# turtle-robotics/sea-current

Measured on AMD Instinct MI355X. Metric: plans/sec (batched start-goal, 1024^2 grid), higher is better.
Workload: dtype int32; 1 GPU; 1024x1024 random-obstacle grids (salt20, one grid and one query block per step), EDT + A*, 1024 batched queries per GPU and step, 10 steps = 10240 queries per library call; queries_per_launch=10240, map=salt20, queries_per_gpu=1024, queries_total=1024, lmax=4096, parallelism=query-sharded x1, contexts_in_flight=2, steps_per_call=10, hw_queues=4

## Files before the change

### sea-current_amd/csrc/astar.hip

```cpp
#include "sc_internal.h"
#include <stdlib.h>

#define NBUCKET 32
#define ASTAR_CQ_THROUGHPUT 1024
#define ASTAR_RU_THROUGHPUT 4
#define ASTAR_CQ_LATENCY 2048
#define ASTAR_RU_LATENCY 8
#define E_RUN (1u << 18)
#define E_START (4u << 13 | 3u << 16)
#define RUNK 8

struct astar_args {
    const uint8_t* moves;
    const int32_t* d2;
    int W, H;
    int32_t rmin;
    const int32_t* start;
    const int32_t* goal;
    const int32_t* qgrid;
    const int32_t* order;
    const int32_t* nq_dev;
    int nq;
    int Lmax;
    int32_t* path;
// ... 11 lines not shown
    int32_t* ovf_sticky;
    int nstat;
    int lazy;
    int tw, bw;
    size_t gcells, bwords;
};

__device__ __forceinline__ int octile(int x, int y, int gx, int gy) {
    int dx = abs(x - gx), dy = abs(y - gy);
    return 10 * max(dx, dy) + 4 * min(dx, dy);
}

__device__ __forceinline__ uint32_t gix(int x, int y, int tw) {
    return ((((uint32_t)(y >> 2) * (uint32_t)tw + (uint32_t)(x >> 2)) << 4) | ((uint32_t)(y & 3) << 2)) | (uint32_t)(x & 3);
}
__device__ __forceinline__ uint32_t gix8(int x, int y, int tw8) {
    return ((((uint32_t)(y >> 3) * (uint32_t)tw8 + (uint32_t)(x >> 3)) << 6) | ((uint32_t)(y & 7) << 3)) | (uint32_t)(x & 7);
}
template <typename GT> __device__ __forceinline__ uint32_t gidx(int x, int y, int tw);
template <> __device__ __forceinline__ uint32_t gidx<uint32_t>(int x, int y, int tw) { return gix(x, y, tw); }
template <> __device__ __forceinline__ uint32_t gidx<uint8_t>(int x, int y, int tw) { return gix8(x, y, tw); }
__device__ __forceinline__ uint32_t cix(int x, int y, int bw) {
    return (((uint32_t)(y >> 4) * (uint32_t)bw + (uint32_t)(x >> 5)) << 4) | (uint32_t)(y & 15);
}

template <typename T>
__device__ __forceinline__ T g_load(const T* p) {
    return __hip_atomic_load(p, __ATOMIC_RELAXED, __HIP_MEMORY_SCOPE_AGENT);
}

__device__ __forceinline__ uint32_t prune_always(int d) {
    const unsigned long long T = 0x75B6D9EA34C851A2ull;
    return (uint32_t)(T >> (8 * d)) & 0xFFu;
}

__device__ __forceinline__ uint32_t entry_pack(int x, int y, int d, uint32_t pmv) {
    const int e0 = (int)((0x6476u >> (4 * (d & 3))) & 7u), e1 = (int)((0x7554u >> (4 * (d & 3))) & 7u);
    const uint32_t side = d < 4 ? (((pmv >> e0) & 1u) | (((pmv >> e1) & 1u) << 1)) : 0u;
// ... 24 lines not shown
                 : "vcc", "scc", "memory");
}
__device__ __forceinline__ void atomic_wait(uint32_t& old) { asm volatile("s_waitcnt vmcnt(0)" : "+v"(old) : : "memory"); }
__device__ __forceinline__ void pop_pair_issue(const uint8_t* mv_addr, uint32_t* bit_addr, uint32_t bits, uint32_t& pmv, uint32_t& old) {
    unsigned long long sv;
    asm volatile("global_load_ubyte %[m], %[ma], off\n\t"
                 "s_mov_b64 %[sv], exec\n\t"
                 "v_cmp_ne_u32_e32 vcc, 0, %[b]\n\t"
                 "s_and_b64 exec, %[sv], vcc\n\t"
                 "global_atomic_or %[o], %[a], %[b], off sc0\n\t"
                 "s_mov_b64 exec, %[sv]"
                 : [sv] "=&s"(sv), [o] "+v"(old), [m] "=&v"(pmv)
                 : [a] "v"(bit_addr), [b] "v"(bits), [ma] "v"(mv_addr)
                 : "vcc", "scc", "memory");
}
__device__ __forceinline__ void pop_run_issue(const uint8_t* const (&ra)[RUNK - 1], const uint8_t* mv_addr, uint32_t* bit_addr, uint32_t bits,
                                              uint32_t (&rm)[RUNK - 1], uint32_t& pmv, uint32_t& old) {
    static_assert(RUNK == 8, "seven run loads are spelled out");
    unsigned long long sv;
    asm volatile("global_load_ubyte %[r0], %[p0], off\n\t"
                 "global_load_ubyte %[r1], %[p1], off\n\t"
                 "global_load_ubyte %[r2], %[p2], off\n\t"
                 "global_load_ubyte %[r3], %[p3], off\n\t"
                 "global_load_ubyte %[r4], %[p4], off\n\t"
                 "global_load_ubyte %[r5], %[p5], off\n\t"
                 "global_load_ubyte %[r6], %[p6], off\n\t"
                 "global_load_ubyte %[m], %[ma], off\n\t"
                 "s_mov_b64 %[sv], exec\n\t"
                 "v_cmp_ne_u32_e32 vcc, 0, %[b]\n\t"
                 "s_and_b64 exec, %[sv], vcc\n\t"
                 "global_atomic_or %[o], %[a], %[b], off sc0\n\t"
                 "s_mov_b64 exec, %[sv]"
                 : [sv] "=&s"(sv), [o] "+v"(old), [m] "=&v"(pmv), [r0] "=&v"(rm[0]), [r1] "=&v"(rm[1]), [r2] "=&v"(rm[2]), [r3] "=&v"(rm[3]),
                   [r4] "=&v"(rm[4]), [r5] "=&v"(rm[5]), [r6] "=&v"(rm[6])
                 : [a] "v"(bit_addr), [b] "v"(bits), [ma] "v"(mv_addr), [p0] "v"(ra[0]), [p1] "v"(ra[1]), [p2] "v"(ra[2]), [p3] "v"(ra[3]),
                   [p4] "v"(ra[4]), [p5] "v"(ra[5]), [p6] "v"(ra[6])
                 : "vcc", "scc", "memory");
}
__device__ __forceinline__ void pop_run_wait_loads(uint32_t (&rm)[RUNK - 1], uint32_t& pmv, uint32_t& old) {
    asm volatile("s_waitcnt vmcnt(1)" : "+v"(pmv), "+v"(old), "+v"(rm[0]), "+v"(rm[1]), "+v"(rm[2]), "+v"(rm[3]), "+v"(rm[4]), "+v"(rm[5]), "+v"(rm[6]) : : "memory");
}
__device__ __forceinline__ void pop_pair_wait_load(uint32_t& pmv, uint32_t& old) { asm volatile("s_waitcnt vmcnt(1)" : "+v"(pmv), "+v"(old) : : "memory"); }

__device__ __forceinline__ void pop_loads_issue(const uint8_t* mv_addr, const uint32_t* w_addr, uint32_t& byte, uint32_t& word) {
    asm volatile("global_load_ubyte %0, %2, off\n\t"
                 "global_load_dword %1, %3, off sc1"
                 : "=&v"(byte), "=&v"(word) : "v"(mv_addr), "v"(w_addr) : "memory");
}
__device__ __forceinline__ void pop_loads_wait(uint32_t& byte, uint32_t& word) { asm volatile("s_waitcnt vmcnt(0)" : "+v"(byte), "+v"(word) : : "memory"); }
__device__ __forceinline__ void masked_or_noret(uint32_t* addr, uint32_t bits) {
// ... 25 lines not shown
    __shared__ uint16_t succ[512];
    __shared__ uint8_t prune_tbl[64];
    __shared__ uint32_t dup_tbl[DUAL ? 1024 + 64 : 1];
    __shared__ uint2 hq_rec[DUAL ? HQ + 64 : 1];
    __shared__ int hq_tail, hq_head, hq_clean, hq_stop, hq_ovf, hq_fcur, hq_found, hq_flush;
    constexpr int SCOPE = DUAL ? __HIP_MEMORY_SCOPE_WORKGROUP : __HIP_MEMORY_SCOPE_WAVEFRONT;
    const int lane = threadIdx.x & 63;
    const int wv = DUAL ? __builtin_amdgcn_readfirstlane((int)(threadIdx.x >> 6)) : 0;
    const int W = a.W, H = a.H;
    const size_t cells = (size_t)W * H;
    const int s = a.start[q], t = a.goal[q];
    int32_t* path = a.path + (size_t)q * a.Lmax;

    int out_st = SC_Q_OK, out_len = 0, out_cost = -1, nexp = 0, npop = 0, kcyc = 0, nstep = 0;
    const size_t grid_off = a.qgrid ? (size_t)a.qgrid[q] * cells : 0;
    const uint8_t* const mvs = a.moves + grid_off;
    const bool bad = s < 0 || t < 0 || (size_t)s >= cells || (size_t)t >= cells || a.d2[grid_off + s] < a.rmin || a.d2[grid_off + t] < a.rmin;
    if (bad) out_st = SC_Q_BAD_ENDPOINT;
    else if (s == t) {
        if (lane == 0 && wv == 0) path[0] = s;
        out_len = 1; out_cost = 0; nexp = 1;
    } else {
    const int tw = a.tw, bw = a.bw;
    GT* g = static_cast<GT*>(a.g) + (size_t)slot * a.gcells;
    uint32_t* cl = a.closed + (size_t)slot * a.bwords;
    uint32_t* bk = a.buckets + (size_t)slot * NBUCKET * a.cap;
    const int cap = a.cap, capm = a.cap - 1;
    const int sx = s % W, sy = s / W, gx = t % W, gy = t / W;
    const int ddx[8] = {1, -1, 0, 0, 1, -1, 1, -1};
    const int ddy[8] = {0, 0, 1, -1, 1, 1, -1, -1};

    {
        uint4* p = reinterpret_cast<uint4*>(cl);
        const size_t n4 = a.bwords >> 2;
        for (size_t i = DUAL ? threadIdx.x : lane; i < n4; i += DUAL ? 128 : 64) p[i] = make_uint4(0, 0, 0, 0);
    }
    __builtin_amdgcn_wave_barrier();
    if (wv == 0 && lane < NBUCKET) { s_head[lane] = 0; s_tail[lane] = 0; }
// ... 5 lines not shown
        qe[0] = (uint32_t)sy << 19 | E_START | (uint32_t)sx;
        hq_tail = 0; hq_head = 0; hq_clean = 0; hq_stop = 0; hq_ovf = 0; hq_fcur = fcur; hq_found = 0; hq_flush = 0;
    }
    asm volatile("s_waitcnt vmcnt(0)" ::: "memory");
    wave_lds_sync();
    if (DUAL) __syncthreads();
    int lh = 0, lt = 1;

    bool found = false, ovf = false;
    const unsigned long long t_begin = __builtin_amdgcn_s_memtime();
    int steps_left = (int)(8 * cells + 1024 < 0x7FFFFFFF ? 8 * cells + 1024 : 0x7FFFFFFF);

    const int mdx = (int)((0x2252u >> (2 * (lane & 7))) & 3u) - 1;
    const int mdy = (int)((0x0A25u >> (2 * (lane & 7))) & 3u) - 1;
    const uint32_t mw = (lane & 7) < 4 ? 10u : 14u;
    const int moff = mdy * W + mdx;

    auto push_entry = [&](const bool act, const uint32_t ne, const int df) {
        const bool same = act && df == 0;
        const unsigned long long m0 = __ballot(same);
        bool spill = false;
        if (m0) {
            const int cnt = __popcll(m0);
            if (__builtin_expect(lt - lh + cnt <= CQ, 1)) {
                if (same) {
                    const int rank = __builtin_amdgcn_mbcnt_hi((uint32_t)(m0 >> 32), __builtin_amdgcn_mbcnt_lo((uint32_t)m0, 0u));
                    qe[(lt + rank) & (CQ - 1)] = ne;
                }
                lt += cnt;
            } else spill = true;
        }
// ... 190 lines not shown
                const int sub = lane >> (kl + 1), j = (lane >> kl) & 1, k = lane & (KL - 1);
                const bool valid = sub < n;
                const uint32_t e_raw = qe[(lh + sub) & (CQ - 1)];
                const uint32_t e = valid ? e_raw : 0u;
                lh += n;
                const int x = e & 0x1FFF, y = e >> 19;
                const uint32_t bit = 1u << (x & 31);
                const int dxg = gx - x, dyg = gy - y, adx = abs(dxg), ady = abs(dyg);
                const int dD = 4 + ((dxg < 0 ? 1 : 0) | (dyg < 0 ? 2 : 0));
                const int dS = adx > ady ? (dxg < 0 ? 1 : 0) : (dyg < 0 ? 3 : 2);
                const uint32_t bD = adx >= 1 && ady >= 1 ? 1u << dD : 0u, bS = adx != ady ? 1u << dS : 0u;
                const int d = j ? dS : dD;
                const bool has = valid && (j ? bS : bD) != 0u;
                const int lgeom = j ? abs(adx - ady) : min(adx, ady);
                const int ddx_ = (int)((0x2252u >> (2 * d)) & 3u) - 1, ddy_ = (int)((0x0A25u >> (2 * d)) & 3u) - 1;
                const uint8_t* const addr = mvs + (y * W + x) + (has ? min(k, lgeom - 1) : 0) * (ddy_ * W + ddx_);
                const bool head = valid && j == 0 && k == 0;
                uint32_t old, byte;
                uint32_t* const wa = &cl[cix(x, y, bw)];
                pop_loads_issue(addr, wa, byte, old);
                const uint32_t prune = prune_tbl[(e >> 13) & 63u];
                const int dup = dup_settle(head, x, y, e);
                pop_loads_wait(byte, old);
                const bool link = has && k < lgeom && ((byte >> d) & 1u) && (k > 0 || !((prune >> d) & 1u));
                const unsigned long long lm = __ballot(link);
                const uint32_t grp = (uint32_t)(lm >> (lane & ~(KL - 1))) & ((1u << KL) - 1u);
                const int run = __ffs((int)~grp) - 1;
                const uint32_t ne = entry_pack(x + (k + 1) * ddx_, y + (k + 1) * ddy_, d, byte) | (k + 1 < run ? E_RUN : 0u);
                const bool won1 = head && dup == 0 && !(old & bit);
                masked_or_noret(wa, won1 ? bit : 0u);
                const unsigned long long wm1 = __ballot(won1);
// ... 12 lines not shown
                nexp += __popcll(wm1);
            } else if (!DUAL && n <= 8) {
                const int sub = lane >> 3, d = lane & 7;
                const bool valid = sub < n;
                const uint32_t e = valid ? qe[(lh + sub) & (CQ - 1)] : 0u;
                lh += n;
                const int x = e & 0x1FFF, y = e >> 19;
                const uint32_t bit = 1u << (x & 31);
                uint32_t old = 0, pmv;
                const int hc = octile(x, y, gx, gy);
                const int nx = x + mdx, ny = y + mdy;
                const int df = (int)mw + octile(nx, ny, gx, gy) - hc;
                const int adx = abs(gx - x), ady = abs(gy - y);
                const int lgeom = d >= 4 ? min(adx, ady) : abs(adx - ady);
                const int lmax = valid && df == 0 ? min(RUNK, lgeom) : 1;
                const uint8_t* const cell = mvs + (y * W + x);
                const uint8_t* ra[RUNK - 1];
                uint32_t rm[RUNK - 1];
#pragma unroll
                for (int k = 1; k < RUNK; ++k) ra[k - 1] = cell + min(k, lmax - 1) * moff;
                pop_run_issue(ra, cell, &cl[cix(x, y, bw)], valid && d == 0 ? bit : 0u, rm, pmv, old);
                const uint32_t prune = prune_tbl[(e >> 13) & 63u];
                pop_run_wait_loads(rm, pmv, old);
                const bool cand = valid && (((pmv & ~prune) >> d) & 1u);
                int run = cand ? 1 : 0;
#pragma unroll
                for (int k = 1; k < RUNK; ++k)
                    if (run == k && k < lmax && ((rm[k - 1] >> d) & 1u)) run = k + 1;
                const uint32_t ne = entry_pack(nx, ny, d, pmv) | (run > 1 ? E_RUN : 0u);
                atomic_wait(old);
                old = bcast_group8(old);
                const bool won = valid && !(old & bit);
                push_entry(won && cand, ne, df);
#pragma unroll
                for (int k = 2; k <= RUNK; ++k) {
                    if (__ballot(won && run >= k) == 0) break;
                    push_entry(won && run >= k, entry_pack(x + k * mdx, y + k * mdy, d, rm[k - 2]) | (run > k ? E_RUN : 0u), 0);
                }
                nexp += __popcll(__ballot(won && d == 0));
                if (__ballot(won && x == gx && y == gy)) found = true;
                if (won && d == 0) g[gidx<GT>(x, y, tw)] = (GT)(fcur - hc);
            } else if (DUAL) {
                const bool valid = lane < n;
                const uint32_t e_raw = qe[(lh + lane) & (CQ - 1)];
                const uint32_t e = valid ? e_raw : 0u;
                lh += n;
                const int x = e & 0x1FFF, y = e >> 19;
                const uint32_t bit = 1u << (x & 31);
                uint32_t old, pmv;
                uint32_t* const wa = &cl[cix(x, y, bw)];
                pop_loads_issue(mvs + (y * W + x), wa, pmv, old);
                const int dup = dup_settle(valid, x, y, e);
                const uint32_t prune = prune_tbl[(e >> 13) & 63u];
                const int dxg = gx - x, dyg = gy - y, adx = abs(dxg), ady = abs(dyg);
                const int dD = 4 + ((dxg < 0 ? 1 : 0) | (dyg < 0 ? 2 : 0));
                const int dS = adx > ady ? (dxg < 0 ? 1 : 0) : (dyg < 0 ? 3 : 2);
                const uint32_t bD = adx >= 1 && ady >= 1 ? 1u << dD : 0u, bS = adx != ady ? 1u << dS : 0u;
                const int nxD = x + (dxg < 0 ? -1 : 1), nyD = y + (dyg < 0 ? -1 : 1);
                const int nxS = x + (adx > ady ? (dxg < 0 ? -1 : 1) : 0), nyS = y + (adx > ady ? 0 : (dyg < 0 ? -1 : 1));
                pop_loads_wait(pmv, old);
                const uint32_t cand = valid ? (pmv & ~prune) : 0u;
                const uint32_t neD = (uint32_t)nyD << 19 | (uint32_t)dD << 13 | (uint32_t)nxD;
                const uint32_t neS = entry_pack(nxS, nyS, dS, pmv);
                const bool won = valid && dup == 0 && !(old & bit);
                masked_or_noret(wa, won ? bit : 0u);
                {
// ... 7 lines not shown
                            lt += c2;
                        } else {
                            push_entry(pD, neD, 0);
                            push_entry(pS, neS, 0);
                        }
                    }
                }
                nexp += __popcll(hand_over(won, x, y, cand & ~(bD | bS), pmv));
            } else {
                const bool valid = lane < n;
                const uint32_t e = valid ? qe[(lh + lane) & (CQ - 1)] : 0u;
                lh += n;
                const int x = e & 0x1FFF, y = e >> 19;
                const uint32_t bit = 1u << (x & 31);
                uint32_t old = 0, pmv;
                pop_pair_issue(mvs + (y * W + x), &cl[cix(x, y, bw)], valid ? bit : 0u, pmv, old);
                const uint32_t prune = prune_tbl[(e >> 13) & 63u];
                const int hc = octile(x, y, gx, gy);
                pop_pair_wait_load(pmv, old);
                uint32_t mv = valid ? (pmv & ~prune) : 0u;
                nd_xy[lane] = (uint32_t)y << 16 | (uint32_t)x;
                nd_mv[lane] = pmv;
                const uint32_t cnt = (uint32_t)__popc(mv);
                int base = 0, total = 0;
#pragma unroll
                for (int bb = 0; bb < 4; ++bb) {
                    const unsigned long long m = __ballot((cnt >> bb) & 1u);
                    base += (int)__builtin_amdgcn_mbcnt_hi((uint32_t)(m >> 32), __builtin_amdgcn_mbcnt_lo((uint32_t)m, 0u)) << bb;
                    total += __popcll(m) << bb;
                }
                while (mv) {
                    const int dd = __ffs((int)mv) - 1;
                    mv &= mv - 1;
                    succ[base++] = (uint16_t)(lane << 3 | dd);
                }
                wave_lds_sync();
                bool won = false;
                for (int j0 = 0; j0 < total; j0 += 64) {
                    const bool act = j0 + lane < total;
                    const uint32_t sd = act ? succ[j0 + lane] : 0u;
                    const int par = (int)(sd >> 3), d = (int)(sd & 7u);
                    const uint32_t xy = nd_xy[par], pmvp = nd_mv[par];
                    const int px = xy & 0xFFFF, py = xy >> 16;
                    const int ddx_ = (int)((0x2252u >> (2 * d)) & 3u) - 1, ddy_ = (int)((0x0A25u >> (2 * d)) & 3u) - 1;
                    const int nx = px + ddx_, ny = py + ddy_;
                    const int df = (d < 4 ? 10 : 14) + octile(nx, ny, gx, gy) - octile(px, py, gx, gy);
                    const uint8_t* ra[RUNK - 1];
#pragma unroll
                    for (int k = 1; k < RUNK; ++k) ra[k - 1] = mvs + (py * W + px);
                    (void)ra;
                    if (j0 == 0) {
                        atomic_wait(old);
                        won = valid && !(old & bit);
                        nexp += __popcll(__ballot(won));
                        if (__ballot(won && x == gx && y == gy)) found = true;
                        nd_mv[lane] = pmv | (won ? 0x100u : 0u);
                        wave_lds_sync();
                    }
                    const bool go = act && ((nd_mv[par] >> 8) & 1u);
                    push_entry(go, entry_pack(nx, ny, d, pmvp), df);
                }
                if (total == 0) {
                    atomic_wait(old);
                    won = valid && !(old & bit);
                    nexp += __popcll(__ballot(won));
// ... 47 lines not shown
        asm volatile("s_waitcnt vmcnt(0)" ::: "memory");
        const int Lmax = a.Lmax;
        int cx = gx, cy = gy, L = 1;
        uint32_t gc = (uint32_t)fcur;
        if (lane == 0) path[Lmax - 1] = t;
        bool broken = false;
        const int wox = lane % 7 - 3, woy = lane / 7 - 3;
        const int md = lane & 7;
        const int mdx_ = (int)((0x2252u >> (2 * md)) & 3u) - 1, mdy_ = (int)((0x0A25u >> (2 * md)) & 3u) - 1;
        const uint32_t mw_ = md < 4 ? 10u : 14u;
        while (!broken && (cx != sx || cy != sy)) {
            uint32_t info = 0u, gw = 0u;
            {
                const int nx = cx + wox, ny = cy + woy;
                if (lane < 49 && nx >= 0 && ny >= 0 && nx < W && ny < H) {
                    const uint32_t mvb = mvs[ny * W + nx];
                    const uint32_t cw = g_load(&cl[cix(nx, ny, bw)]);
                    gw = (uint32_t)g_load(&g[gidx<GT>(nx, ny, tw)]);
                    info = mvb | ((cw >> (nx & 31)) & 1u) << 8;
                }
            }
            int ox = 0, oy = 0;
            for (int k = 0; k < 3 && !broken && (cx != sx || cy != sy); ++k) {
                const int src = (oy - mdy_ + 3) * 7 + (ox - mdx_ + 3);
                const uint32_t ni = (uint32_t)__shfl((int)info, src, 64), ng = (uint32_t)__shfl((int)gw, src, 64);
                const bool ok = lane < 8 && ((ni >> md) & 1u) && ((ni >> 8) & 1u) && (GT)ng == (GT)(gc - mw_);
                const unsigned long long m = __ballot(ok);
                if (!m) broken = true;
                else {
                    const int d = __ffsll((long long)m) - 1;
                    cx -= ddx[d]; cy -= ddy[d];
// ... 115 lines not shown
    if (const char* e = getenv("SC_ASTAR_DUAL")) { const int v = atoi(e); if (v == 0) n = 0; else if (v > 1 && v < n) n = v; }
    if (latency) { if (const char* e = getenv("SC_ASTAR_LATENCY")) { if (atoi(e) == 0) n = 0; } }
    cached = n;
    return n;
}

static int astar_run(sc_ctx* ctx, const int32_t* d2, int G, const int32_t* qgrid, int W, int H, int32_t r2, const int32_t* start,
                     const int32_t* goal, int Q, int Lmax, int32_t* path, int32_t* len, int32_t* cost,
                     int32_t* status, bool full_g = false) {
    const size_t cells = (size_t)W * H;
    const int tw = full_g ? (W + 3) >> 2 : (W + 7) >> 3, bw = (W + 31) >> 5;
    const size_t gcells = full_g ? (size_t)tw * ((H + 3) >> 2) * 16 : (size_t)tw * ((H + 7) >> 3) * 64;
    const size_t gsz = full_g ? 4 : 1;
    const size_t bwords = (size_t)bw * ((H + 15) >> 4) * 16;
    const int32_t rmin = r2 > 1 ? r2 : 1;
    int r = sc_scratch_reserve(ctx, &ctx->moves, cells * (size_t)G);
    if (r != SC_OK) return r;
    r = sc_launch_moves(ctx, d2, W, H * G, H, r2, (uint8_t*)ctx->moves.p);
    if (r != SC_OK) return r;
    r = sc_scratch_reserve(ctx, &ctx->qstats, (size_t)Q * 6 * sizeof(int32_t));
    if (r != SC_OK) return r;
    int32_t* expanded = (int32_t*)ctx->qstats.p;
    int32_t* order = expanded + 4 * (size_t)Q;
    int32_t* ovf_list = order + Q;
    ctx->last_Q = Q;
    int cap = ctx->astar_cap;
    if (const char* e = getenv("SC_ASTAR_CAP")) { const int v = atoi(e); if (v >= 1024 && (v & (v - 1)) == 0) cap = v; }
    if (cells > ((size_t)1 << 21)) {
        int want = 1 << 15;
        while (want < 64 * (W > H ? W : H)) want <<= 1;
        if (cap < want) cap = want;
    }
    const size_t per_slot = gcells * gsz + bwords * 4 + (size_t)NBUCKET * cap * 4;
// ... 60 lines not shown
extern "C" int sc_astar_batch(sc_ctx* ctx, const int32_t* d2, int W, int H, int32_t r2_clear,
                              const int32_t* start, const int32_t* goal, int Q, int Lmax,
                              int32_t* path, int32_t* len, int32_t* cost, int32_t* status) {
    if (!ctx || !d2 || !start || !goal || !path || !len || !cost || !status || W <= 0 || H <= 0 || Q < 0 ||
        Lmax <= 0 || W > SC_MAX_DIM || H > SC_MAX_DIM)
        return SC_ERR_INVALID;
    if (Q == 0) return SC_OK;
    SC_HIP(ctx, hipSetDevice(ctx->device));
    return astar_run(ctx, d2, 1, nullptr, W, H, r2_clear, start, goal, Q, Lmax, path, len, cost, status);
}

extern "C" int sc_astar_batch_multi(sc_ctx* ctx, const int32_t* d2, int G, const int32_t* qgrid, int W, int H, int32_t r2_clear,
                                    const int32_t* start, const int32_t* goal, int Q, int Lmax,
                                    int32_t* path, int32_t* len, int32_t* cost, int32_t* status) {
    if (!ctx || !d2 || !qgrid || !start || !goal || !path || !len || !cost || !status || G <= 0 || W <= 0 || H <= 0 || Q < 0 ||
        Lmax <= 0 || W > SC_MAX_DIM || H > SC_MAX_DIM || (long long)H * G > 0x7FFFFFFF / (W > 0 ? W : 1))
        return SC_ERR_INVALID;
    if (Q == 0) return SC_OK;
    SC_HIP(ctx, hipSetDevice(ctx->device));
    return astar_run(ctx, d2, G, qgrid, W, H, r2_clear, start, goal, Q, Lmax, path, len, cost, status);
}

extern "C" int sc_astar_last_expansions(sc_ctx* ctx, int64_t* expansions) {
    if (!ctx || !expansions) return SC_ERR_INVALID;
    *expansions = 0;
    if (ctx->last_Q <= 0) return SC_OK;
    std::vector<int32_t> ex(ctx->last_Q);
    SC_HIP(ctx, hipMemcpyAsync(ex.data(), ctx->qstats.p, (size_t)ctx->last_Q * 4, hipMemcpyDeviceToHost, ctx->stream));
    SC_HIP(ctx, hipStreamSynchronize(ctx->stream));
    int64_t tot = 0;
    for (int v : ex) tot += v;
// ... 41 lines not shown
```

### sea-current_amd/csrc/moves.hip

```cpp
#include "sc_internal.h"

__global__ void __launch_bounds__(256)
moves_kernel(const int32_t* __restrict__ d2, int W, int Hall, int H, int32_t rmin, uint8_t* __restrict__ moves) {
    const int x = blockIdx.x * 256 + threadIdx.x;
    const int yall = blockIdx.y;
    if (x >= W) return;
    const int y = yall % H;
    const int32_t* r1 = d2 + (size_t)yall * W;
    bool t[3][3];
#pragma unroll
    for (int j = -1; j <= 1; ++j)
#pragma unroll
        for (int i = -1; i <= 1; ++i) {
            int xx = x + i, yy = y + j;
            t[j + 1][i + 1] = xx >= 0 && xx < W && yy >= 0 && yy < H && r1[(ptrdiff_t)j * W + xx] >= rmin;
        }
    uint32_t m = 0;
    if (t[1][1]) {
        m |= (uint32_t)t[1][2] << 0;
        m |= (uint32_t)t[1][0] << 1;
        m |= (uint32_t)t[2][1] << 2;
        m |= (uint32_t)t[0][1] << 3;
        m |= (uint32_t)(t[2][2] && t[1][2] && t[2][1]) << 4;
        m |= (uint32_t)(t[2][0] && t[1][0] && t[2][1]) << 5;
        m |= (uint32_t)(t[0][2] && t[1][2] && t[0][1]) << 6;
        m |= (uint32_t)(t[0][0] && t[1][0] && t[0][1]) << 7;
    }
    moves[(size_t)yall * W + x] = (uint8_t)m;
}

__global__ void __launch_bounds__(256)
moves4_kernel(const int32_t* __restrict__ d2, int W, int Hall, int H, int32_t rmin, uint8_t* __restrict__ moves) {
    const int x = 4 * (blockIdx.x * 256 + threadIdx.x);
    const int yall = blockIdx.y;
    if (x >= W) return;
    const int y = yall % H;
    const int32_t* r1 = d2 + (size_t)yall * W;
    uint32_t t[3] = {0u, 0u, 0u};
#pragma unroll
    for (int j = -1; j <= 1; ++j) {
        const int yy = y + j;
        if (yy < 0 || yy >= H) continue;
        const int32_t* r = r1 + (ptrdiff_t)j * W;
        const int4 v = *reinterpret_cast<const int4*>(r + x);
        const int32_t l = x > 0 ? r[x - 1] : 0, q = x + 4 < W ? r[x + 4] : 0;
        t[j + 1] = (uint32_t)(l >= rmin) | (uint32_t)(v.x >= rmin) << 1 | (uint32_t)(v.y >= rmin) << 2 | (uint32_t)(v.z >= rmin) << 3 |
                   (uint32_t)(v.w >= rmin) << 4 | (uint32_t)(q >= rmin) << 5;
    }
    uint32_t out = 0;
#pragma unroll
    for (int i = 0; i < 4; ++i) {
        const uint32_t a = t[0] >> i, c = t[1] >> i, b = t[2] >> i;
        uint32_t m = 0;
        if (c & 2u) {
            const uint32_t E = (c >> 2) & 1u, Wt = c & 1u, S = (b >> 1) & 1u, N = (a >> 1) & 1u;
            m = E | Wt << 1 | S << 2 | N << 3 | (((b >> 2) & 1u) & E & S) << 4 | ((b & 1u) & Wt & S) << 5 | (((a >> 2) & 1u) & E & N) << 6 |
                ((a & 1u) & Wt & N) << 7;
        }
        out |= m << (8 * i);
    }
    *reinterpret_cast<uint32_t*>(moves + (size_t)yall * W + x) = out;
}

__global__ void __launch_bounds__(256)
moves4x4_kernel(const int32_t* __restrict__ d2, int W, int Hall, int H, int32_t rmin, uint8_t* __restrict__ moves) {
    const int x = 4 * (blockIdx.x * 256 + threadIdx.x);
    const int yall0 = 4 * blockIdx.y;
    if (x >= W) return;
    const int y0 = yall0 % H;
    const int32_t* r1 = d2 + (size_t)yall0 * W;
    uint32_t t[6];
#pragma unroll
    for (int j = 0; j < 6; ++j) {
        const int yy = y0 + j - 1;
        t[j] = 0u;
        if (yy < 0 || yy >= H) continue;
        const int32_t* r = r1 + (ptrdiff_t)(j - 1) * W;
        const int4 v = *reinterpret_cast<const int4*>(r + x);
        const int32_t l = x > 0 ? r[x - 1] : 0, q = x + 4 < W ? r[x + 4] : 0;
        t[j] = (uint32_t)(l >= rmin) | (uint32_t)(v.x >= rmin) << 1 | (uint32_t)(v.y >= rmin) << 2 | (uint32_t)(v.z >= rmin) << 3 |
               (uint32_t)(v.w >= rmin) << 4 | (uint32_t)(q >= rmin) << 5;
    }
#pragma unroll
    for (int k = 0; k < 4; ++k) {
        uint32_t out = 0;
#pragma unroll
        for (int i = 0; i < 4; ++i) {
            const uint32_t a = t[k] >> i, c = t[k + 1] >> i, b = t[k + 2] >> i;
            uint32_t m = 0;
            if (c & 2u) {
                const uint32_t E = (c >> 2) & 1u, Wt = c & 1u, S = (b >> 1) & 1u, N = (a >> 1) & 1u;
                m = E | Wt << 1 | S << 2 | N << 3 | (((b >> 2) & 1u) & E & S) << 4 | ((b & 1u) & Wt & S) << 5 | (((a >> 2) & 1u) & E & N) << 6 |
                    ((a & 1u) & Wt & N) << 7;
            }
            out |= m << (8 * i);
        }
        *reinterpret_cast<uint32_t*>(moves + (size_t)(yall0 + k) * W + x) = out;
    }
}

int sc_launch_moves(sc_ctx* ctx, const int32_t* d2, int W, int Hall, int H, int32_t r2, uint8_t* moves) {
    int32_t rmin = r2 > 1 ? r2 : 1;
    int tk = sc_time_begin(ctx, SC_K_MOVES);
    if (W % 4 == 0 && H % 4 == 0 && ((uintptr_t)d2 & 15) == 0 && ((uintptr_t)moves & 3) == 0)
        hipLaunchKernelGGL(moves4x4_kernel, dim3((W / 4 + 255) / 256, Hall / 4), dim3(256), 0, ctx->stream, d2, W, Hall, H, rmin, moves);
    else if (W % 4 == 0 && ((uintptr_t)d2 & 15) == 0 && ((uintptr_t)moves & 3) == 0)
        hipLaunchKernelGGL(moves4_kernel, dim3((W / 4 + 255) / 256, Hall), dim3(256), 0, ctx->stream, d2, W, Hall, H, rmin, moves);
    else
        hipLaunchKernelGGL(moves_kernel, dim3((W + 255) / 256, Hall), dim3(256), 0, ctx->stream, d2, W, Hall, H, rmin, moves);
    sc_time_end(ctx, tk);
    SC_HIP(ctx, hipGetLastError());
    return SC_OK;
}

extern "C" int sc_moves_i32_u8(sc_ctx* ctx, const int32_t* d2, int W, int H, int32_t r2_clear, uint8_t* moves) {
    if (!ctx || !d2 || !moves || W <= 0 || H <= 0 || W > SC_MAX_DIM || H > SC_MAX_DIM) return SC_ERR_INVALID;
    SC_HIP(ctx, hipSetDevice(ctx->device));
    return sc_launch_moves(ctx, d2, W, H, H, r2_clear, moves);
}

__host__ __device__ static inline int64_t isqrt64(int64_t v) {
    int64_t r = (int64_t)sqrt((double)v);
    while (r * r > v) --r;
    while ((r + 1) * (r + 1) <= v) ++r;
    return r;
}

__global__ void __launch_bounds__(256)
clearance_penalty_kernel(const int32_t* __restrict__ d2, size_t n, int32_t thr, int32_t r2_soft, int64_t s10, int pen_max,
                         uint8_t* __restrict__ pen) {
    const size_t i = (size_t)blockIdx.x * 256 + threadIdx.x;
    if (i >= n) return;
    const int32_t d = d2[i];
    uint8_t p = 0;
    if (d >= thr && d < r2_soft) p = (uint8_t)(((int64_t)pen_max * (s10 - isqrt64(100ll * d))) / s10);
// ... 33 lines not shown
```

### sea-current_amd/csrc/sc_internal.h

```cpp
#pragma once
#include <hip/hip_runtime.h>
#include <math.h>
#include <stdint.h>
#include <stdio.h>
#include <string.h>

#include <set>
#include <vector>

#include "../../include/sea_current_hip.h"

struct sc_scratch {
    void* p = nullptr;
    size_t bytes = 0;
    sc_scratch() = default;
    sc_scratch(const sc_scratch&) = delete;
    sc_scratch& operator=(const sc_scratch&) = delete;
    ~sc_scratch() { if (p) (void)hipFree(p); }
};

static inline size_t al256(size_t b) { return (b + 255) & ~(size_t)255; }

enum sc_status_word {
    SC_ST_ASTAR_OVERFLOW,
// ... 131 lines not shown
        end_ += al256(bytes ? bytes : 1);
        return (int)off_.size() - 1;
    }
    sc_ctx* ctx_;
    size_t end_ = 0;
    std::vector<size_t> off_;
    std::vector<copy> up_, down_;
};

int sc_time_begin(sc_ctx* ctx, int kid);
void sc_time_end(sc_ctx* ctx, int token);
int sc_time_chain(sc_ctx* ctx, int token, int kid);

int sc_launch_edt(sc_ctx* ctx, const uint8_t* occ, int W, int H, int batch, int32_t* d2);
int sc_launch_moves(sc_ctx* ctx, const int32_t* d2, int W, int Hall, int H, int32_t r2, uint8_t* moves);
int sc_launch_arclength(sc_ctx* ctx, const float* ctrl, int S, int nsub, float* cum, float* seg_len, const int32_t* S_dev);
int sc_launch_resample(sc_ctx* ctx, const float* ctrl, const float* cum, const float* arclength, const int32_t* seg_off, int B, int S,
                       int nsub, float* profile_pos, const int32_t* prof_off, int nudge, float* pts, float* tpar, int32_t* seg,
                       float* curvature, int32_t* status, const int32_t* S_dev);
struct sc_speed_frame {
    const int32_t* d2;
    int W, H;
    float x_min, y_min, res_x, res_y;
};
static inline bool sc_frame_ok(const sc_speed_frame& fr) {
    return fr.W >= 1 && fr.W <= SC_MAX_DIM && fr.H >= 1 && fr.H <= SC_MAX_DIM && isfinite(fr.x_min) && isfinite(fr.y_min) &&
           isfinite(fr.res_x) && fr.res_x > 0.f && isfinite(fr.res_y) && fr.res_y > 0.f;
}
int sc_launch_speed_limits(sc_ctx* ctx, const float* ctrl, const float* cum, const int32_t* seg_off, const float* arclength,
                           const int32_t* status, int P, int nsub, int N, int J, const double* limits, const double* dyn,
// ... 39 lines not shown
```

Measured before the change: 745,400 plans/s.

## Store A* move masks in 8x8 tiled layout with SGPR-based run loads

The per-cell move-mask array is now written by new tiled moves kernels in an 8x8-tile layout, and every A* access to it (pops, runs, jump probes, path window) goes through the tile index. Run loads in the jump path now use a scalar base address plus 32-bit per-lane offsets. The aim is better cache-line locality for the spatially clustered reads of A* expansion and diagonal runs, and fewer address VGPRs. In exchange each access pays extra index arithmetic, the array is padded to whole tiles, and an s_nop is added before the loads.

```diff
diff --git a/sea-current_amd/csrc/astar.hip b/sea-current_amd/csrc/astar.hip
--- a/sea-current_amd/csrc/astar.hip
+++ b/sea-current_amd/csrc/astar.hip
@@ -49,14 +49,12 @@
 __device__ __forceinline__ uint32_t gix(int x, int y, int tw) {
     return ((((uint32_t)(y >> 2) * (uint32_t)tw + (uint32_t)(x >> 2)) << 4) | ((uint32_t)(y & 3) << 2)) | (uint32_t)(x & 3);
 }
-__device__ __forceinline__ uint32_t gix8(int x, int y, int tw8) {
-    return ((((uint32_t)(y >> 3) * (uint32_t)tw8 + (uint32_t)(x >> 3)) << 6) | ((uint32_t)(y & 7) << 3)) | (uint32_t)(x & 7);
-}
+__device__ __forceinline__ uint32_t gix8(int x, int y, int tw8) { return sc_tile8_ix(x, y, tw8); }
 template <typename GT> __device__ __forceinline__ uint32_t gidx(int x, int y, int tw);
 template <> __device__ __forceinline__ uint32_t gidx<uint32_t>(int x, int y, int tw) { return gix(x, y, tw); }
 template <> __device__ __forceinline__ uint32_t gidx<uint8_t>(int x, int y, int tw) { return gix8(x, y, tw); }
 __device__ __forceinline__ uint32_t cix(int x, int y, int bw) {
-    return (((uint32_t)(y >> 4) * (uint32_t)bw + (uint32_t)(x >> 5)) << 4) | (uint32_t)(y & 15);
+    return ((__umul24((uint32_t)y >> 4, (uint32_t)bw) + ((uint32_t)x >> 5)) << 4) | ((uint32_t)y & 15u);
 }
 
 template <typename T>
@@ -111,18 +109,21 @@
                  : [a] "v"(bit_addr), [b] "v"(bits), [ma] "v"(mv_addr)
                  : "vcc", "scc", "memory");
 }
-__device__ __forceinline__ void pop_run_issue(const uint8_t* const (&ra)[RUNK - 1], const uint8_t* mv_addr, uint32_t* bit_addr, uint32_t bits,
+__device__ __forceinline__ void pop_run_issue(const uint8_t* base, const uint32_t (&ra)[RUNK - 1], uint32_t mv_off, uint32_t* bit_addr, uint32_t bits,
                                               uint32_t (&rm)[RUNK - 1], uint32_t& pmv, uint32_t& old) {
     static_assert(RUNK == 8, "seven run loads are spelled out");
     unsigned long long sv;
-    asm volatile("global_load_ubyte %[r0], %[p0], off\n\t"
-                 "global_load_ubyte %[r1], %[p1], off\n\t"
-                 "global_load_ubyte %[r2], %[p2], off\n\t"
-                 "global_load_ubyte %[r3], %[p3], off\n\t"
-                 "global_load_ubyte %[r4], %[p4], off\n\t"
-                 "global_load_ubyte %[r5], %[p5], off\n\t"
-                 "global_load_ubyte %[r6], %[p6], off\n\t"
-                 "global_load_ubyte %[m], %[ma], off\n\t"
+    const unsigned long long mb = (unsigned long long)(uint32_t)__builtin_amdgcn_readfirstlane((int)(uint32_t)(uintptr_t)base) |
+                                  (unsigned long long)(uint32_t)__builtin_amdgcn_readfirstlane((int)(uint32_t)((uintptr_t)base >> 32)) << 32;
+    asm volatile("s_nop 4\n\t"
+                 "global_load_ubyte %[r0], %[p0], %[mb]\n\t"
+                 "global_load_ubyte %[r1], %[p1], %[mb]\n\t"
+                 "global_load_ubyte %[r2], %[p2], %[mb]\n\t"
+                 "global_load_ubyte %[r3], %[p3], %[mb]\n\t"
+                 "global_load_ubyte %[r4], %[p4], %[mb]\n\t"
+                 "global_load_ubyte %[r5], %[p5], %[mb]\n\t"
+                 "global_load_ubyte %[r6], %[p6], %[mb]\n\t"
+                 "global_load_ubyte %[m], %[ma], %[mb]\n\t"
                  "s_mov_b64 %[sv], exec\n\t"
                  "v_cmp_ne_u32_e32 vcc, 0, %[b]\n\t"
                  "s_and_b64 exec, %[sv], vcc\n\t"
@@ -130,7 +131,7 @@
                  "s_mov_b64 exec, %[sv]"
                  : [sv] "=&s"(sv), [o] "+v"(old), [m] "=&v"(pmv), [r0] "=&v"(rm[0]), [r1] "=&v"(rm[1]), [r2] "=&v"(rm[2]), [r3] "=&v"(rm[3]),
                    [r4] "=&v"(rm[4]), [r5] "=&v"(rm[5]), [r6] "=&v"(rm[6])
-                 : [a] "v"(bit_addr), [b] "v"(bits), [ma] "v"(mv_addr), [p0] "v"(ra[0]), [p1] "v"(ra[1]), [p2] "v"(ra[2]), [p3] "v"(ra[3]),
+                 : [a] "v"(bit_addr), [b] "v"(bits), [mb] "s"(mb), [ma] "v"(mv_off), [p0] "v"(ra[0]), [p1] "v"(ra[1]), [p2] "v"(ra[2]), [p3] "v"(ra[3]),
                    [p4] "v"(ra[4]), [p5] "v"(ra[5]), [p6] "v"(ra[6])
                  : "vcc", "scc", "memory");
 }
@@ -186,7 +187,7 @@
 
     int out_st = SC_Q_OK, out_len = 0, out_cost = -1, nexp = 0, npop = 0, kcyc = 0, nstep = 0;
     const size_t grid_off = a.qgrid ? (size_t)a.qgrid[q] * cells : 0;
-    const uint8_t* const mvs = a.moves + grid_off;
+    const uint8_t* const mvs = a.moves + (a.qgrid ? (size_t)a.qgrid[q] * a.gcells : 0);
     const bool bad = s < 0 || t < 0 || (size_t)s >= cells || (size_t)t >= cells || a.d2[grid_off + s] < a.rmin || a.d2[grid_off + t] < a.rmin;
     if (bad) out_st = SC_Q_BAD_ENDPOINT;
     else if (s == t) {
@@ -194,6 +195,7 @@
         out_len = 1; out_cost = 0; nexp = 1;
     } else {
     const int tw = a.tw, bw = a.bw;
+    const int mtw = sizeof(GT) == 1 ? tw : (W + 7) >> 3;
     GT* g = static_cast<GT*>(a.g) + (size_t)slot * a.gcells;
     uint32_t* cl = a.closed + (size_t)slot * a.bwords;
     uint32_t* bk = a.buckets + (size_t)slot * NBUCKET * a.cap;
@@ -229,7 +231,6 @@
     const int mdx = (int)((0x2252u >> (2 * (lane & 7))) & 3u) - 1;
     const int mdy = (int)((0x0A25u >> (2 * (lane & 7))) & 3u) - 1;
     const uint32_t mw = (lane & 7) < 4 ? 10u : 14u;
-    const int moff = mdy * W + mdx;
 
     auto push_entry = [&](const bool act, const uint32_t ne, const int df) {
         const bool same = act && df == 0;
@@ -450,7 +451,8 @@
                 const bool has = valid && (j ? bS : bD) != 0u;
                 const int lgeom = j ? abs(adx - ady) : min(adx, ady);
                 const int ddx_ = (int)((0x2252u >> (2 * d)) & 3u) - 1, ddy_ = (int)((0x0A25u >> (2 * d)) & 3u) - 1;
-                const uint8_t* const addr = mvs + (y * W + x) + (has ? min(k, lgeom - 1) : 0) * (ddy_ * W + ddx_);
+                const int kc = has ? min(k, lgeom - 1) : 0;
+                const uint8_t* const addr = mvs + gix8(x + __mul24(kc, ddx_), y + __mul24(kc, ddy_), mtw);
                 const bool head = valid && j == 0 && k == 0;
                 uint32_t old, byte;
                 uint32_t* const wa = &cl[cix(x, y, bw)];
@@ -493,12 +495,15 @@
                 const int adx = abs(gx - x), ady = abs(gy - y);
                 const int lgeom = d >= 4 ? min(adx, ady) : abs(adx - ady);
                 const int lmax = valid && df == 0 ? min(RUNK, lgeom) : 1;
-                const uint8_t* const cell = mvs + (y * W + x);
-                const uint8_t* ra[RUNK - 1];
+                const uint32_t cell = gix8(x, y, mtw);
+                uint32_t ra[RUNK - 1];
                 uint32_t rm[RUNK - 1];
 #pragma unroll
-                for (int k = 1; k < RUNK; ++k) ra[k - 1] = cell + min(k, lmax - 1) * moff;
-                pop_run_issue(ra, cell, &cl[cix(x, y, bw)], valid && d == 0 ? bit : 0u, rm, pmv, old);
+                for (int k = 1; k < RUNK; ++k) {
+                    const int kc = min(k, lmax - 1);
+                    ra[k - 1] = gix8(x + __mul24(kc, mdx), y + __mul24(kc, mdy), mtw);
+                }
+                pop_run_issue(mvs, ra, cell, &cl[cix(x, y, bw)], valid && d == 0 ? bit : 0u, rm, pmv, old);
                 const uint32_t prune = prune_tbl[(e >> 13) & 63u];
                 pop_run_wait_loads(rm, pmv, old);
                 const bool cand = valid && (((pmv & ~prune) >> d) & 1u);
@@ -528,7 +533,7 @@
                 const uint32_t bit = 1u << (x & 31);
                 uint32_t old, pmv;
                 uint32_t* const wa = &cl[cix(x, y, bw)];
-                pop_loads_issue(mvs + (y * W + x), wa, pmv, old);
+                pop_loads_issue(mvs + gix8(x, y, mtw), wa, pmv, old);
                 const int dup = dup_settle(valid, x, y, e);
                 const uint32_t prune = prune_tbl[(e >> 13) & 63u];
                 const int dxg = gx - x, dyg = gy - y, adx = abs(dxg), ady = abs(dyg);
@@ -566,7 +571,7 @@
                 const int x = e & 0x1FFF, y = e >> 19;
                 const uint32_t bit = 1u << (x & 31);
                 uint32_t old = 0, pmv;
-                pop_pair_issue(mvs + (y * W + x), &cl[cix(x, y, bw)], valid ? bit : 0u, pmv, old);
+                pop_pair_issue(mvs + gix8(x, y, mtw), &cl[cix(x, y, bw)], valid ? bit : 0u, pmv, old);
                 const uint32_t prune = prune_tbl[(e >> 13) & 63u];
                 const int hc = octile(x, y, gx, gy);
                 pop_pair_wait_load(pmv, old);
@@ -597,10 +602,6 @@
                     const int ddx_ = (int)((0x2252u >> (2 * d)) & 3u) - 1, ddy_ = (int)((0x0A25u >> (2 * d)) & 3u) - 1;
                     const int nx = px + ddx_, ny = py + ddy_;
                     const int df = (d < 4 ? 10 : 14) + octile(nx, ny, gx, gy) - octile(px, py, gx, gy);
-                    const uint8_t* ra[RUNK - 1];
-#pragma unroll
-                    for (int k = 1; k < RUNK; ++k) ra[k - 1] = mvs + (py * W + px);
-                    (void)ra;
                     if (j0 == 0) {
                         atomic_wait(old);
                         won = valid && !(old & bit);
@@ -678,7 +679,7 @@
             {
                 const int nx = cx + wox, ny = cy + woy;
                 if (lane < 49 && nx >= 0 && ny >= 0 && nx < W && ny < H) {
-                    const uint32_t mvb = mvs[ny * W + nx];
+                    const uint32_t mvb = mvs[gix8(nx, ny, mtw)];
                     const uint32_t cw = g_load(&cl[cix(nx, ny, bw)]);
                     gw = (uint32_t)g_load(&g[gidx<GT>(nx, ny, tw)]);
                     info = mvb | ((cw >> (nx & 31)) & 1u) << 8;
@@ -824,9 +825,10 @@
     const size_t gsz = full_g ? 4 : 1;
     const size_t bwords = (size_t)bw * ((H + 15) >> 4) * 16;
     const int32_t rmin = r2 > 1 ? r2 : 1;
-    int r = sc_scratch_reserve(ctx, &ctx->moves, cells * (size_t)G);
+    const size_t mcells = (size_t)((W + 7) >> 3) * ((H + 7) >> 3) * 64;
+    int r = sc_scratch_reserve(ctx, &ctx->moves, mcells * (size_t)G);
     if (r != SC_OK) return r;
-    r = sc_launch_moves(ctx, d2, W, H * G, H, r2, (uint8_t*)ctx->moves.p);
+    r = sc_launch_moves_tiled(ctx, d2, W, H, G, r2, (uint8_t*)ctx->moves.p);
     if (r != SC_OK) return r;
     r = sc_scratch_reserve(ctx, &ctx->qstats, (size_t)Q * 6 * sizeof(int32_t));
     if (r != SC_OK) return r;
@@ -917,7 +919,8 @@
                                     const int32_t* start, const int32_t* goal, int Q, int Lmax,
                                     int32_t* path, int32_t* len, int32_t* cost, int32_t* status) {
     if (!ctx || !d2 || !qgrid || !start || !goal || !path || !len || !cost || !status || G <= 0 || W <= 0 || H <= 0 || Q < 0 ||
-        Lmax <= 0 || W > SC_MAX_DIM || H > SC_MAX_DIM || (long long)H * G > 0x7FFFFFFF / (W > 0 ? W : 1))
+        Lmax <= 0 || W > SC_MAX_DIM || H > SC_MAX_DIM ||
+        (long long)G * (((H + 7) >> 3) * 8) > 0x7FFFFFFF / (((W + 7) >> 3) * 8))
         return SC_ERR_INVALID;
     if (Q == 0) return SC_OK;
     SC_HIP(ctx, hipSetDevice(ctx->device));
diff --git a/sea-current_amd/csrc/moves.hip b/sea-current_amd/csrc/moves.hip
--- a/sea-current_amd/csrc/moves.hip
+++ b/sea-current_amd/csrc/moves.hip
@@ -1,19 +1,13 @@
 #include "sc_internal.h"
 
-__global__ void __launch_bounds__(256)
-moves_kernel(const int32_t* __restrict__ d2, int W, int Hall, int H, int32_t rmin, uint8_t* __restrict__ moves) {
-    const int x = blockIdx.x * 256 + threadIdx.x;
-    const int yall = blockIdx.y;
-    if (x >= W) return;
-    const int y = yall % H;
-    const int32_t* r1 = d2 + (size_t)yall * W;
+__device__ __forceinline__ uint32_t mcell_mask(const int32_t* g0, int W, int H, int x, int y, int32_t rmin) {
     bool t[3][3];
 #pragma unroll
     for (int j = -1; j <= 1; ++j)
 #pragma unroll
         for (int i = -1; i <= 1; ++i) {
-            int xx = x + i, yy = y + j;
-            t[j + 1][i + 1] = xx >= 0 && xx < W && yy >= 0 && yy < H && r1[(ptrdiff_t)j * W + xx] >= rmin;
+            const int xx = x + i, yy = y + j;
+            t[j + 1][i + 1] = xx >= 0 && xx < W && yy >= 0 && yy < H && g0[(ptrdiff_t)yy * W + xx] >= rmin;
         }
     uint32_t m = 0;
     if (t[1][1]) {
@@ -26,31 +20,21 @@
         m |= (uint32_t)(t[0][2] && t[1][2] && t[0][1]) << 6;
         m |= (uint32_t)(t[0][0] && t[1][0] && t[0][1]) << 7;
     }
-    moves[(size_t)yall * W + x] = (uint8_t)m;
-}
-
-__global__ void __launch_bounds__(256)
-moves4_kernel(const int32_t* __restrict__ d2, int W, int Hall, int H, int32_t rmin, uint8_t* __restrict__ moves) {
-    const int x = 4 * (blockIdx.x * 256 + threadIdx.x);
-    const int yall = blockIdx.y;
-    if (x >= W) return;
-    const int y = yall % H;
-    const int32_t* r1 = d2 + (size_t)yall * W;
-    uint32_t t[3] = {0u, 0u, 0u};
-#pragma unroll
-    for (int j = -1; j <= 1; ++j) {
-        const int yy = y + j;
-        if (yy < 0 || yy >= H) continue;
-        const int32_t* r = r1 + (ptrdiff_t)j * W;
-        const int4 v = *reinterpret_cast<const int4*>(r + x);
-        const int32_t l = x > 0 ? r[x - 1] : 0, q = x + 4 < W ? r[x + 4] : 0;
-        t[j + 1] = (uint32_t)(l >= rmin) | (uint32_t)(v.x >= rmin) << 1 | (uint32_t)(v.y >= rmin) << 2 | (uint32_t)(v.z >= rmin) << 3 |
-                   (uint32_t)(v.w >= rmin) << 4 | (uint32_t)(q >= rmin) << 5;
-    }
+    return m;
+}
+__device__ __forceinline__ uint32_t mrow_bits(const int32_t* g0, int W, int H, int x, int yy, int32_t rmin) {
+    if (yy < 0 || yy >= H) return 0u;
+    const int32_t* r = g0 + (size_t)yy * W;
+    const int4 v = *reinterpret_cast<const int4*>(r + x);
+    const int32_t l = x > 0 ? r[x - 1] : 0, q = x + 4 < W ? r[x + 4] : 0;
+    return (uint32_t)(l >= rmin) | (uint32_t)(v.x >= rmin) << 1 | (uint32_t)(v.y >= rmin) << 2 | (uint32_t)(v.z >= rmin) << 3 |
+           (uint32_t)(v.w >= rmin) << 4 | (uint32_t)(q >= rmin) << 5;
+}
+__device__ __forceinline__ uint32_t mrow_masks(uint32_t ta, uint32_t tc, uint32_t tb) {
     uint32_t out = 0;
 #pragma unroll
     for (int i = 0; i < 4; ++i) {
-        const uint32_t a = t[0] >> i, c = t[1] >> i, b = t[2] >> i;
+        const uint32_t a = ta >> i, c = tc >> i, b = tb >> i;
         uint32_t m = 0;
         if (c & 2u) {
             const uint32_t E = (c >> 2) & 1u, Wt = c & 1u, S = (b >> 1) & 1u, N = (a >> 1) & 1u;
@@ -59,7 +43,29 @@
         }
         out |= m << (8 * i);
     }
-    *reinterpret_cast<uint32_t*>(moves + (size_t)yall * W + x) = out;
+    return out;
+}
+
+__global__ void __launch_bounds__(256)
+moves_kernel(const int32_t* __restrict__ d2, int W, int Hall, int H, int32_t rmin, uint8_t* __restrict__ moves) {
+    const int x = blockIdx.x * 256 + threadIdx.x;
+    const int yall = blockIdx.y;
+    if (x >= W) return;
+    const int y = yall % H;
+    moves[(size_t)yall * W + x] = (uint8_t)mcell_mask(d2 + (size_t)(yall - y) * W, W, H, x, y, rmin);
+}
+
+__global__ void __launch_bounds__(256)
+moves4_kernel(const int32_t* __restrict__ d2, int W, int Hall, int H, int32_t rmin, uint8_t* __restrict__ moves) {
+    const int x = 4 * (blockIdx.x * 256 + threadIdx.x);
+    const int yall = blockIdx.y;
+    if (x >= W) return;
+    const int y = yall % H;
+    const int32_t* g0 = d2 + (size_t)(yall - y) * W;
+    uint32_t t[3];
+#pragma unroll
+    for (int j = 0; j < 3; ++j) t[j] = mrow_bits(g0, W, H, x, y + j - 1, rmin);
+    *reinterpret_cast<uint32_t*>(moves + (size_t)yall * W + x) = mrow_masks(t[0], t[1], t[2]);
 }
 
 __global__ void __launch_bounds__(256)
@@ -68,35 +74,12 @@
     const int yall0 = 4 * blockIdx.y;
     if (x >= W) return;
     const int y0 = yall0 % H;
-    const int32_t* r1 = d2 + (size_t)yall0 * W;
+    const int32_t* g0 = d2 + (size_t)(yall0 - y0) * W;
     uint32_t t[6];
 #pragma unroll
-    for (int j = 0; j < 6; ++j) {
-        const int yy = y0 + j - 1;
-        t[j] = 0u;
-        if (yy < 0 || yy >= H) continue;
-        const int32_t* r = r1 + (ptrdiff_t)(j - 1) * W;
-        const int4 v = *reinterpret_cast<const int4*>(r + x);
-        const int32_t l = x > 0 ? r[x - 1] : 0, q = x + 4 < W ? r[x + 4] : 0;
-        t[j] = (uint32_t)(l >= rmin) | (uint32_t)(v.x >= rmin) << 1 | (uint32_t)(v.y >= rmin) << 2 | (uint32_t)(v.z >= rmin) << 3 |
-               (uint32_t)(v.w >= rmin) << 4 | (uint32_t)(q >= rmin) << 5;
-    }
-#pragma unroll
-    for (int k = 0; k < 4; ++k) {
-        uint32_t out = 0;
-#pragma unroll
-        for (int i = 0; i < 4; ++i) {
-            const uint32_t a = t[k] >> i, c = t[k + 1] >> i, b = t[k + 2] >> i;
-            uint32_t m = 0;
-            if (c & 2u) {
-                const uint32_t E = (c >> 2) & 1u, Wt = c & 1u, S = (b >> 1) & 1u, N = (a >> 1) & 1u;
-                m = E | Wt << 1 | S << 2 | N << 3 | (((b >> 2) & 1u) & E & S) << 4 | ((b & 1u) & Wt & S) << 5 | (((a >> 2) & 1u) & E & N) << 6 |
-                    ((a & 1u) & Wt & N) << 7;
-            }
-            out |= m << (8 * i);
-        }
-        *reinterpret_cast<uint32_t*>(moves + (size_t)(yall0 + k) * W + x) = out;
-    }
+    for (int j = 0; j < 6; ++j) t[j] = mrow_bits(g0, W, H, x, y0 + j - 1, rmin);
+#pragma unroll
+    for (int k = 0; k < 4; ++k) *reinterpret_cast<uint32_t*>(moves + (size_t)(yall0 + k) * W + x) = mrow_masks(t[k], t[k + 1], t[k + 2]);
 }
 
 int sc_launch_moves(sc_ctx* ctx, const int32_t* d2, int W, int Hall, int H, int32_t r2, uint8_t* moves) {
@@ -119,6 +102,73 @@
     return sc_launch_moves(ctx, d2, W, H, H, r2_clear, moves);
 }
 
+__global__ void __launch_bounds__(256)
+moves_tiled_kernel(const int32_t* __restrict__ d2, int W, int H, int tw8, size_t tcells, int32_t rmin, uint8_t* __restrict__ moves) {
+    const int x = blockIdx.x * 256 + threadIdx.x, y = blockIdx.y;
+    if (x >= 8 * tw8) return;
+    const uint32_t m = x < W && y < H ? mcell_mask(d2 + (size_t)blockIdx.z * H * W, W, H, x, y, rmin) : 0u;
+    moves[(size_t)blockIdx.z * tcells + sc_tile8_ix(x, y, tw8)] = (uint8_t)m;
+}
+
+__global__ void __launch_bounds__(256)
+moves4_tiled_kernel(const int32_t* __restrict__ d2, int W, int H, int tw8, size_t tcells, int32_t rmin, uint8_t* __restrict__ moves) {
+    const int x = 4 * (blockIdx.x * 256 + threadIdx.x), y = blockIdx.y;
+    if (x >= 8 * tw8) return;
+    const int32_t* g0 = d2 + (size_t)blockIdx.z * H * W;
+    uint32_t out = 0;
+    if (x < W && y < H) {
+        uint32_t t[3];
+#pragma unroll
+        for (int j = 0; j < 3; ++j) t[j] = mrow_bits(g0, W, H, x, y + j - 1, rmin);
+        out = mrow_masks(t[0], t[1], t[2]);
+    }
+    *reinterpret_cast<uint32_t*>(moves + (size_t)blockIdx.z * tcells + sc_tile8_ix(x, y, tw8)) = out;
+}
+
+__global__ void __launch_bounds__(256)
+moves4x4_tiled_kernel(const int32_t* __restrict__ d2, int W, int H, int tw8, size_t tcells, int32_t rmin, uint8_t* __restrict__ moves) {
+    const int x = 4 * (blockIdx.x * 256 + threadIdx.x), y0 = 4 * blockIdx.y;
+    if (x >= 8 * tw8) return;
+    const int32_t* g0 = d2 + (size_t)blockIdx.z * H * W;
+    const bool in = x < W && y0 < H;
+    uint32_t t[6];
+#pragma unroll
+    for (int j = 0; j < 6; ++j) t[j] = in ? mrow_bits(g0, W, H, x, y0 + j - 1, rmin) : 0u;
+    uint8_t* const o = moves + (size_t)blockIdx.z * tcells + sc_tile8_ix(x, y0, tw8);
+#pragma unroll
+    for (int k = 0; k < 4; ++k) *reinterpret_cast<uint32_t*>(o + 8 * k) = in ? mrow_masks(t[k], t[k + 1], t[k + 2]) : 0u;
+}
+
+int sc_launch_moves_tiled(sc_ctx* ctx, const int32_t* d2, int W, int H, int G, int32_t r2, uint8_t* moves) {
+    const int32_t rmin = r2 > 1 ? r2 : 1;
+    const int tw8 = (W + 7) >> 3, th8 = (H + 7) >> 3;
+    const size_t tcells = (size_t)tw8 * th8 * 64;
+    const bool al = W % 4 == 0 && ((uintptr_t)d2 & 15) == 0 && ((uintptr_t)moves & 3) == 0;
+    int tk = sc_time_begin(ctx, SC_K_MOVES);
+    for (int g0 = 0; g0 < G; g0 += 65535) {
+        const unsigned gz = (unsigned)(G - g0 < 65535 ? G - g0 : 65535);
+        const int32_t* d = d2 + (size_t)g0 * H * W;
+        uint8_t* m = moves + (size_t)g0 * tcells;
+        if (al && H % 4 == 0)
+            hipLaunchKernelGGL(moves4x4_tiled_kernel, dim3((2 * tw8 + 255) / 256, 2 * th8, gz), dim3(256), 0, ctx->stream, d, W, H, tw8, tcells, rmin, m);
+        else if (al)
+            hipLaunchKernelGGL(moves4_tiled_kernel, dim3((2 * tw8 + 255) / 256, 8 * th8, gz), dim3(256), 0, ctx->stream, d, W, H, tw8, tcells, rmin, m);
+        else
+            hipLaunchKernelGGL(moves_tiled_kernel, dim3((8 * tw8 + 255) / 256, 8 * th8, gz), dim3(256), 0, ctx->stream, d, W, H, tw8, tcells, rmin, m);
+    }
+    sc_time_end(ctx, tk);
+    SC_HIP(ctx, hipGetLastError());
+    return SC_OK;
+}
+
+extern "C" int sc_moves_tiled_i32_u8(sc_ctx* ctx, const int32_t* d2, int W, int H, int G, int32_t r2_clear, uint8_t* out) {
+    if (!ctx || !d2 || !out || W <= 0 || H <= 0 || G <= 0 || W > SC_MAX_DIM || H > SC_MAX_DIM ||
+        (long long)G * (((H + 7) >> 3) * 8) > 0x7FFFFFFF / (((W + 7) >> 3) * 8))
+        return SC_ERR_INVALID;
+    SC_HIP(ctx, hipSetDevice(ctx->device));
+    return sc_launch_moves_tiled(ctx, d2, W, H, G, r2_clear, out);
+}
+
 __host__ __device__ static inline int64_t isqrt64(int64_t v) {
     int64_t r = (int64_t)sqrt((double)v);
     while (r * r > v) --r;
diff --git a/sea-current_amd/csrc/sc_internal.h b/sea-current_amd/csrc/sc_internal.h
--- a/sea-current_amd/csrc/sc_internal.h
+++ b/sea-current_amd/csrc/sc_internal.h
@@ -169,6 +169,11 @@
 
 int sc_launch_edt(sc_ctx* ctx, const uint8_t* occ, int W, int H, int batch, int32_t* d2);
 int sc_launch_moves(sc_ctx* ctx, const int32_t* d2, int W, int Hall, int H, int32_t r2, uint8_t* moves);
+__device__ __forceinline__ uint32_t sc_tile8_ix(int x, int y, int tw8) {
+    return ((__umul24((uint32_t)y >> 3, (uint32_t)tw8) + ((uint32_t)x >> 3)) << 6) | (((uint32_t)y & 7u) << 3) | ((uint32_t)x & 7u);
+}
+int sc_launch_moves_tiled(sc_ctx* ctx, const int32_t* d2, int W, int H, int G, int32_t r2, uint8_t* moves);
+extern "C" int sc_moves_tiled_i32_u8(sc_ctx* ctx, const int32_t* d2, int W, int H, int G, int32_t r2_clear, uint8_t* out);
 int sc_launch_arclength(sc_ctx* ctx, const float* ctrl, int S, int nsub, float* cum, float* seg_len, const int32_t* S_dev);
 int sc_launch_resample(sc_ctx* ctx, const float* ctrl, const float* cum, const float* arclength, const int32_t* seg_off, int B, int S,
                        int nsub, float* profile_pos, const int32_t* prof_off, int nudge, float* pts, float* tpar, int32_t* seg,
```

Measured after the change: 765,900 plans/s (median of 6 runs). 2.8% higher.
